# loyer-yuan/GeneralSparse

Hardware: AMD Instinct MI355X
Metric: SpMM GFLOP/s + achieved HBM GB/s vs rocSPARSE, pruned-weight fp16 N=32 (higher is better)
Workload: dtype f16 (fp32 accumulate)

## Files before the change

generalsparse_amd/autotune.py:

```python
import math

CANDIDATES = {
    "f16": [("block_total", 20, 1), ("block_total", 10, 1), ("block_total", 40, 1), ("block_total", 80, 1),
            ("block_total", 40, 1, {"KS_NT": 1}), ("block_total", 80, 1, {"KS_NT": 1}),
            ("tblock_warp_total", 20, 2), ("tblock_warp_total", 24, 2), ("tblock_warp_total", 4, 1),
            ("warp_segment", 4, 1), ("thread_total", 4, 1)],
    "f16_2to4": [("col_direction_nm", 32, 1), ("col_direction_nm", 32, 1, {"NM_NT": 0}),
                 ("col_direction_nm", 32, 1, {"NM_TILES": 8})],
    "f32": [("thread_total", 4, 1), ("tblock_warp_total", 4, 1), ("tblock_warp_total", 32, 8),
            ("tblock_warp_total", 32, 16), ("tblock_warp_total", 64, 16), ("merge_path", 512, 1)],
    "f32_powerlaw": [("merge_path", 256, 1), ("merge_path", 512, 1), ("merge_path", 1024, 1),
                     ("balanced_block_total", 2048, 1), ("thread_total", 4, 1)],
    "f32_powerlaw_large": [("merge_path", 512, 1), ("merge_path", 1024, 1), ("merge_path", 2048, 1),
                           ("merge_path", 1024, 1, {"MP_COL_PARTS": 4}), ("merge_path", 2048, 1, {"MP_COL_PARTS": 2})],
}
F32_EXTRA = {"f16": [("tblock_warp_total", 64, 8), ("tblock_warp_total", 72, 8)]}
WORKLOAD_CLASS = {"c1": "f32", "c2": "f16", "c3": "f16_2to4", "c4": "f32_powerlaw", "c4o": "f32_powerlaw_large"}


def row_block_rows(M, cus=256, max_rows=64):
    rounds = max(1, math.ceil(M / (cus * max_rows)))
    return max(1, math.ceil(M / (cus * rounds)))


def shape_candidates(M):
    rb = row_block_rows(M)
    return [("tblock_warp_total", rb, 2, {"KS_MIN_ROWS": 1000}), ("block_total", 56, 1, {}),
            ("block_total", 40, 1, {}), ("block_total", 80, 1, {}), ("block_total", 112, 1, {})]


def candidates_for(M, K, nnz, dtype, two_four=False, powerlaw=False):
    if dtype in ("f16", "bf16"):
        if two_four:
            return list(CANDIDATES["f16_2to4"])
        c = list(CANDIDATES["f16"])
        rb = ("tblock_warp_total", row_block_rows(M), 2)
        if rb not in c:
            c.append(rb)
        return c
    if powerlaw:
        return list(CANDIDATES["f32_powerlaw_large" if nnz > 50_000_000 else "f32_powerlaw"])
    return list(CANDIDATES["f32"]) + [c for c in F32_EXTRA["f16"] if c not in CANDIDATES["f32"]]


def cand_key(c):
    return "%s(%d,%d)%s" % (c[0], c[1], c[2], "".join(f" {a}={b}" for a, b in (c[3] if len(c) > 3 else {}).items()))


def build_candidate(M, K, row, col, val, cand, N, dtype, device=0):
    from . import Plan, get_config, set_config
    name, p0, p1 = cand[:3]
    over = cand[3] if len(cand) > 3 else {}
    old = {k: get_config(k) for k in over}
    try:
        for k, v in over.items():
            set_config(k, v)
        plan = Plan.from_coo(M, K, row, col, val).run_pipeline(name, N, p0, p1).compile()
        plan.upload(dtype, device)
    finally:
        for k, v in old.items():
            set_config(k, v)
    return plan


def autotune(M, K, row, col, val, N, dtype="f16", candidates=None, device=0, reps=50, rotation_mb=640.0,
             save_path=None, two_four=False, powerlaw=False, rounds=3):
    import torch
    from . import GsError
    tdt = {"f16": torch.float16, "bf16": torch.bfloat16}.get(dtype, torch.float32)
    e = 2 if dtype in ("f16", "bf16") else 4
    dev = torch.device(f"cuda:{device}")
    if candidates is None:
        candidates = candidates_for(M, K, len(row), dtype, two_four=two_four, powerlaw=powerlaw)
    results, built = {}, []
    for cand in candidates:
        key = cand_key(cand)
        try:
            plan = build_candidate(M, K, row, col, val, cand, N, dtype, device)
        except GsError as ex:
            results[key] = str(ex)
            continue
        copies = max(2, int(math.ceil(rotation_mb * 1e6 / (plan.info()["device_bytes_A"] + K * N * e))))
        for _ in range(copies - 1):
            plan.add_replica()
        Bs = [torch.randn((K, N), device=dev, dtype=tdt) for _ in range(copies)]
        Cs = [torch.empty((M, N), device=dev, dtype=tdt) for _ in range(copies)]
        built.append([key, plan, plan.rotation(Bs, Cs), Bs, Cs, []])
    for _ in range(max(1, rounds)):
        for b in built:
            rot = b[2]
            rot.run(5, 0)
            torch.cuda.synchronize(dev)
            e0, e1 = torch.cuda.Event(enable_timing=True), torch.cuda.Event(enable_timing=True)
            e0.record()
            rot.run(reps, 0)
            e1.record()
            torch.cuda.synchronize(dev)
            b[5].append(e0.elapsed_time(e1) / reps * 1e3)
    best = None
    for b in built:
        us = sorted(b[5])[len(b[5]) // 2]
        results[b[0]] = round(us, 3)
        if best is None or us < best[0]:
            best = (us, b)
    if best is None:
        raise GsError("no candidate plan could be built")
    for b in built:
        b[2] = b[3] = b[4] = None
        if b is not best[1]:
            b[1].free()
    plan = best[1][1]
    if save_path:
        plan.save(save_path)
    return plan, results
```

generalsparse_amd/csrc/hip_code/kernel_common.hpp:

```cpp
#pragma once

#include <hip/hip_fp16.h>
#include <hip/hip_runtime.h>
#include <stdint.h>

#include <type_traits>

#include "idx_formula.hpp"
#include "kernel_consts.hpp"

namespace gsk {

typedef _Float16 f16;
typedef __bf16 bf16;
typedef unsigned int u32x4 __attribute__((ext_vector_type(4)));
typedef unsigned int u32x2 __attribute__((ext_vector_type(2)));

template <int BYTES> struct raw_vec;
template <> struct raw_vec<2> { typedef uint16_t t; };
template <> struct raw_vec<4> { typedef uint32_t t; };
template <> struct raw_vec<8> { typedef uint2 t; };
template <> struct raw_vec<16> { typedef uint4 t; };
struct alignas(16) u32x8 { uint4 lo, hi; };
template <> struct raw_vec<32> { typedef u32x8 t; };

template <class VT, int CF>
__device__ __forceinline__ void load_f32(const VT *__restrict__ p, float (&out)[CF]) {
    typedef typename raw_vec<CF * sizeof(VT)>::t R;
    R r = *reinterpret_cast<const R *>(p);
    VT tmp[CF];
    __builtin_memcpy(tmp, &r, sizeof(R));
#pragma unroll
    for (int k = 0; k < CF; k++) out[k] = (float)tmp[k];
}

template <class VT, int CF>
__device__ __forceinline__ void store_f32(VT *__restrict__ p, const float (&in)[CF]) {
    typedef typename raw_vec<CF * sizeof(VT)>::t R;
    VT tmp[CF];
#pragma unroll
    for (int k = 0; k < CF; k++) tmp[k] = (VT)in[k];
    R r;
    __builtin_memcpy(&r, tmp, sizeof(R));
    *reinterpret_cast<R *>(p) = r;
}

template <class T>
__device__ __forceinline__ T ld_once(const T *p) {
#if defined(GS_A_NT) && GS_A_NT
    return __builtin_nontemporal_load(p);
#else
    return *p;
#endif
}
template <bool NT, class T>
__device__ __forceinline__ T ld_once_if(const T *p) {
    if constexpr (NT) return __builtin_nontemporal_load(p);
    else return ld_once(p);
}
template <int BYTES> struct raw_ext;
template <> struct raw_ext<1> { typedef uint8_t t; };
template <> struct raw_ext<2> { typedef uint16_t t; };
template <> struct raw_ext<4> { typedef uint32_t t; };
template <> struct raw_ext<8> { typedef u32x2 t; };
template <> struct raw_ext<16> { typedef u32x4 t; };

template <class T, int SCF>
__device__ __forceinline__ void load_raw(const T *__restrict__ p, T (&out)[SCF]) {
    if constexpr (SCF * sizeof(T) <= 16) {
        typedef typename raw_ext<SCF * sizeof(T)>::t R;
        R r = ld_once(reinterpret_cast<const R *>(p));
        __builtin_memcpy(out, &r, sizeof(R));
    } else {
        static_assert(SCF * sizeof(T) == 32, "8 to 32 bytes");
        u32x4 r[2] = {ld_once(reinterpret_cast<const u32x4 *>(p)), ld_once(reinterpret_cast<const u32x4 *>(p) + 1)};
        __builtin_memcpy(out, r, 32);
    }
}

template <int CF>
__device__ __forceinline__ void wave_reduce_slots(float (&acc)[CF], int X) {
    for (int off = X; off < 64; off <<= 1) {
#pragma unroll
        for (int k = 0; k < CF; k++) acc[k] += __shfl_xor(acc[k], off, 64);
    }
}

template <class VT, int CF>
__device__ __forceinline__ void atomic_add_vals(VT *p, const float (&v)[CF]);

template <>
__device__ __forceinline__ void atomic_add_vals<float, 1>(float *p, const float (&v)[1]) {
    unsafeAtomicAdd(p, v[0]);
}
template <>
__device__ __forceinline__ void atomic_add_vals<float, 4>(float *p, const float (&v)[4]) {
#pragma unroll
    for (int k = 0; k < 4; k++) unsafeAtomicAdd(p + k, v[k]);
}
template <>
__device__ __forceinline__ void atomic_add_vals<float, 8>(float *p, const float (&v)[8]) {
#pragma unroll
    for (int k = 0; k < 8; k++) unsafeAtomicAdd(p + k, v[k]);
}
template <>
__device__ __forceinline__ void atomic_add_vals<f16, 8>(f16 *p, const float (&v)[8]) {
#pragma unroll
    for (int k = 0; k < 8; k += 2) {
        __half2 h = __floats2half2_rn(v[k], v[k + 1]);
        unsafeAtomicAdd(reinterpret_cast<__half2 *>(p + k), h);
    }
}
template <>
__device__ __forceinline__ void atomic_add_vals<f16, 1>(f16 *p, const float (&v)[1]) {
    unsafeAtomicAdd(reinterpret_cast<__half *>(p), __float2half(v[0]));
}

__device__ __forceinline__ uint32_t xcd_block(uint32_t b, uint32_t n) {
#ifdef GS_NO_XCD_SWIZZLE
    return b;
#endif
    const uint32_t q = n >> 3, r = n & 7u, x = b & 7u;
    return (x < r ? x * (q + 1u) : r * (q + 1u) + (x - r) * q) + (b >> 3);
}

template <class VT, int CF>
__device__ __forceinline__ void fma_row(float (&acc)[CF], float v, const VT *__restrict__ brow) {
    float b[CF];
    load_f32<VT, CF>(brow, b);
#pragma unroll
    for (int k = 0; k < CF; k++) acc[k] = __builtin_fmaf(v, b[k], acc[k]);
}

typedef _Float16 h8v __attribute__((ext_vector_type(8)));
typedef short s4v __attribute__((ext_vector_type(4)));
typedef float f4v __attribute__((ext_vector_type(4)));
typedef __attribute__((address_space(3))) s4v lds_s4v;
typedef _Float16 h16v __attribute__((ext_vector_type(16)));
typedef __bf16 b8v __attribute__((ext_vector_type(8)));
template <class ET> struct mfma_elem;
template <> struct mfma_elem<f16> {
    typedef h8v frag;
    static __device__ __forceinline__ f4v mfma_16x16x32(const frag &a, const frag &b, const f4v &c) {
        return __builtin_amdgcn_mfma_f32_16x16x32_f16(a, b, c, 0, 0, 0);
    }
};
template <> struct mfma_elem<bf16> {
    typedef b8v frag;
    static __device__ __forceinline__ f4v mfma_16x16x32(const frag &a, const frag &b, const f4v &c) {
        return __builtin_amdgcn_mfma_f32_16x16x32_bf16(a, b, c, 0, 0, 0);
    }
};
typedef uint32_t u32x2_a2 __attribute__((ext_vector_type(2), aligned(2)));

template <int CT>
__device__ __forceinline__ uint32_t b_piece(uint32_t k, uint32_t p) {
    uint32_t sw;
    if constexpr (CT == 1) sw = 0;
    else if constexpr (CT == 2) sw = (k >> 3) & 1u;
    else if constexpr (CT == 4) sw = ((k >> 1) & 1u) | (((k >> 3) & 1u) << 1);
    else sw = (k & 3u) | (((k >> 3) & 1u) << 2);
    return p ^ (sw & (uint32_t)(CT - 1));
}

__device__ __forceinline__ u32x4 ks_slab_wait(const uint32_t *src, uint32_t tag, uint32_t *err, bool force) {
    u32x4 w;
    auto load4 = [&]() {
#pragma unroll
        for (int i = 0; i < 4; i++) w[i] = __hip_atomic_load(src + i, __ATOMIC_RELAXED, __HIP_MEMORY_SCOPE_AGENT);
    };
    auto stale = [&]() { return (((w[0] ^ tag) | (w[1] ^ tag) | (w[2] ^ tag) | (w[3] ^ tag)) & 1u) != 0u; };
    bool lost = force;
    if (!lost) {
        load4();
        if (stale()) {
            uint64_t t0 = __builtin_amdgcn_s_memrealtime(), prev = t0;
            uint32_t polls = 0;
            do {
                const uint64_t t = __builtin_amdgcn_s_memrealtime();
                if (t - prev > 100000ull) {
                    t0 = t;
                    polls = 0;
                }
                prev = t;
                if (t - t0 > 20000000ull && polls >= 1024u) {
                    lost = true;
                    break;
                }
                polls++;
                __builtin_amdgcn_s_sleep(2);
                load4();
            } while (stale());
        }
    }
    if (lost) {
        w = u32x4{0x7fc00000u | tag, 0x7fc00000u | tag, 0x7fc00000u | tag, 0x7fc00000u | tag};
        __hip_atomic_fetch_or(err, 1u, __ATOMIC_RELAXED, __HIP_MEMORY_SCOPE_AGENT);
    }
    return w;
}
#ifdef GS_EXPERIMENTS
#define GS_KS_FORCE(prio) (((prio) & 16u) != 0u)
#else
#define GS_KS_FORCE(prio) false
#endif

}
```

generalsparse_amd/csrc/hip_code/mfma_ks.hpp:

```cpp
#pragma once

#include "kernel_common.hpp"

namespace gsk {

template <int N>
__device__ constexpr int vmcnt_imm() {
    static_assert(N >= 0 && N < 64, "vmcnt is six bits");
    return (N & 0xF) | ((N >> 4) << 14) | 0x70 | 0xF00;
}


#ifndef GS_KS_FULL_TILE
#define GS_KS_FULL_TILE 1
#endif
enum : int { kKsPosU16 = 0, kKsPos8 = 1, kKsPosWin = 2 };
template <int CT, int RT, int W, int D, int MAXG, bool STAMPS, bool AP = true, int PF = kKsPosU16, int NTL = 0, class ET = f16>
__device__ __forceinline__ void ks_body(const uint32_t *__restrict__ bmtb_first_row, const u32x4 *__restrict__ tP,
                                        const u32x4 *__restrict__ tV, const u32x2 *__restrict__ steps,
                                        const ET *__restrict__ B, ET *__restrict__ C, uint32_t K, uint32_t N, uint32_t S,
                                        uint32_t NS, uint32_t nwg, uint32_t row_base, float *__restrict__ slabs,
                                        uint32_t *__restrict__ arrivals, uint64_t *__restrict__ stamps, uint32_t bx,
                                        uint32_t prio, const uint8_t *__restrict__ tW = nullptr) {
    constexpr bool P8 = PF == kKsPos8, WP = PF == kKsPosWin;
    constexpr uint32_t RB = 32 * CT;
    constexpr uint32_t UB = 2 * CT;
    constexpr uint32_t IMG = ks_image_bytes<RT>();
    constexpr uint32_t STG = 32u * RB;
    extern __shared__ __attribute__((aligned(16))) unsigned char lds[];
    const uint32_t tid = threadIdx.x, lane = tid & 63u;
    const uint32_t wv = __builtin_amdgcn_readfirstlane(tid >> 6);
    const uint32_t u = xcd_block(bx, nwg);
    const uint32_t g = u / S, q = u - g * S;
#define GS_KS_STAMP(slot)                                                                          \
    if constexpr (STAMPS) {                                                                        \
        if (lane == 0) stamps[((size_t)blockIdx.x * W + wv) * 32u + (slot)] = __builtin_amdgcn_s_memtime(); \
    }
    GS_KS_STAMP(0u);
    const uint32_t k0 = q * NS * 32u;
    const uint32_t col0 = blockIdx.y * 16u * CT, nv = min(16u * CT, N - col0);
    unsigned char *img = lds + wv * (IMG + STG);
    unsigned char *bst = img + IMG;
    const u32x4 zero4 = {0u, 0u, 0u, 0u};

    const uint32_t nsw = NS > wv ? (NS - wv + W - 1u) / W : 0u;
    const size_t ubase = (size_t)u * NS;
    using PV = typename std::conditional<P8 || WP, u32x2, u32x4>::type;
    const PV *tPp = reinterpret_cast<const PV *>(tP);
    PV P[D][MAXG];
    u32x4 V[D][MAXG], BR[D][CT];
    uint32_t WN[D][MAXG];
    u32x2 NX[D];
    uint32_t CN[D];
    uint32_t vz;
    __asm__ volatile("v_mov_b32 %0, 0" : "=v"(vz));
    auto rec_of = [&](uint32_t i) -> u32x2 {
        const uint32_t st = __builtin_amdgcn_readfirstlane(i < nsw ? wv + i * W : 0u);
        return steps[ubase + st + vz];
    };
    uint32_t boff[CT];
#pragma unroll
    for (int c = 0; c < CT; c++) boff[c] = ((lane + 64u * c) / UB) * N + ((lane + 64u * c) % UB) * 8u;
    auto load_b = [&](auto fast, uint32_t i, u32x4 (&B_)[CT]) {
        const uint32_t st = __builtin_amdgcn_readfirstlane(i < nsw ? wv + i * W : 0u);
        const uint32_t kr = k0 + st * 32u;
        if constexpr (decltype(fast)::value) {
            const ET *Bk = B + (size_t)kr * N + col0;
#pragma unroll
            for (int c = 0; c < CT; c++) B_[c] = ld_once_if<(NTL & 2) != 0>(reinterpret_cast<const u32x4 *>(Bk + boff[c]));
            return;
        }
#pragma unroll
        for (int c = 0; c < CT; c++) {
            const uint32_t un = lane + 64u * c;
            const uint32_t k = kr + un / UB, cu = (un % UB) * 8u;
            B_[c] = ld_once_if<(NTL & 2) != 0>(
                reinterpret_cast<const u32x4 *>(B + (size_t)(k < K ? k : K - 1u) * N + col0 + (cu < nv ? cu : 0u)));
        }
    };
    auto load_g_at = [&](uint32_t i, uint32_t b0, uint32_t gc, u32x2 &NX_, uint32_t &CN_, PV (&P_)[MAXG],
                         u32x4 (&V_)[MAXG], uint32_t (&W_)[MAXG]) {
        CN_ = gc;
        NX_ = rec_of(i + D);
#pragma unroll
        for (int j = 0; j < MAXG; j++) {
            const uint32_t qg = lane + 64u * j;
            const size_t at = (size_t)b0 + (qg < gc ? qg : 0u);
            P_[j] = ld_once_if<(NTL & 1) != 0>(tPp + at);
            V_[j] = ld_once_if<(NTL & 1) != 0>(tV + at);
            if constexpr (WP) W_[j] = ld_once_if<(NTL & 1) != 0>(tW + at);
        }
    };
    auto load_g = [&](uint32_t i, u32x2 &NX_, uint32_t &CN_, PV (&P_)[MAXG], u32x4 (&V_)[MAXG], uint32_t (&W_)[MAXG]) {
        load_g_at(i, __builtin_amdgcn_readfirstlane(NX_[0]), __builtin_amdgcn_readfirstlane(NX_[1]), NX_, CN_, P_, V_, W_);
    };
    const uint32_t GH = (prio >> 8) & 0x3ffu;
    if (GH) {
#pragma unroll
        for (int d = 0; d < D; d++) load_b(std::false_type{}, (uint32_t)d, BR[d]);
#pragma unroll
        for (int d = 0; d < D; d++) {
            const uint32_t st = (uint32_t)d < nsw ? wv + (uint32_t)d * W : 0u;
            load_g_at((uint32_t)d, (u * min((uint32_t)(W * D), NS) + st) * GH, GH, NX[d], CN[d], P[d], V[d], WN[d]);
        }
        for (uint32_t x = lane; x < IMG / 16u; x += 64u) *reinterpret_cast<u32x4 *>(img + x * 16u) = zero4;
    } else {
#pragma unroll
        for (int d = 0; d < D; d++) NX[d] = rec_of((uint32_t)d);
#pragma unroll
        for (int d = 0; d < D; d++) load_b(std::false_type{}, (uint32_t)d, BR[d]);
        for (uint32_t x = lane; x < IMG / 16u; x += 64u) *reinterpret_cast<u32x4 *>(img + x * 16u) = zero4;
#pragma unroll
        for (int d = 0; d < D; d++) load_g((uint32_t)d, NX[d], CN[d], P[d], V[d], WN[d]);
    }
    GS_KS_STAMP(1u);

    f4v acc[RT][CT];
#pragma unroll
    for (int rt = 0; rt < RT; rt++)
#pragma unroll
        for (int ct = 0; ct < CT; ct++) acc[rt][ct] = f4v{0.f, 0.f, 0.f, 0.f};
    uint32_t arow[RT];
#pragma unroll
    for (int rt = 0; rt < RT; rt++) arow[rt] = (16u * rt + (lane & 15u)) * kKsStride + 16u * (lane >> 4);

    auto ent_h = [&](const PV &p, uint32_t hb, int e) -> uint32_t {
        if constexpr (P8) {
            const uint32_t b = (p[e >> 2] >> (8 * (e & 3))) & 0x7fu;
            return hb + 48u * (b >> 4) + (b & 15u);
        } else {
            return (p[e >> 1] >> (16 * (e & 1))) & 0xffffu;
        }
    };
    auto grp_hb = [&](const PV &p) -> uint32_t {
        if constexpr (P8) {
            const uint32_t x = p[0], y = p[1];
            const uint32_t sg = ((x >> 7) & 1u) | ((x >> 14) & 2u) | ((x >> 21) & 4u) | ((x >> 28) & 8u) | ((y >> 3) & 16u);
            return 384u * (sg >> 1) + 16u * (sg & 1u);
        } else {
            return 0u;
        }
    };
    auto step = [&](auto fast, uint32_t i, u32x2 &NX_, uint32_t &CN_, PV (&P_)[MAXG], u32x4 (&V_)[MAXG], u32x4 (&B_)[CT],
                    uint32_t (&W_)[MAXG]) {
        const bool live = i < nsw;
        const uint32_t gc = CN_;
        typedef typename mfma_elem<ET>::frag frag;
        frag av[RT], bv[CT];
        if (live) {
            const uint32_t kr = k0 + (wv + i * W) * 32u;
#pragma unroll
            for (int c = 0; c < CT; c++) {
                const uint32_t un = lane + 64u * c, k = un / UB, s = un % UB;
                u32x4 b = B_[c];
                if constexpr (!decltype(fast)::value) b = kr + k < K && s * 8u < nv ? b : zero4;
                *reinterpret_cast<u32x4 *>(bst + k * RB + b_piece<CT>(k, s >> 1) * 32u + (s & 1u) * 16u) = b;
            }
            unsigned char *wa[WP ? MAXG : 1][8];
            if constexpr (WP) {
#pragma unroll
                for (int j = 0; j < MAXG; j++) {
                    unsigned char *wb = img + W_[j] * 480u;
#pragma unroll
                    for (int e = 0; e < 8; e++) wa[j][e] = wb + 2u * ((P_[j][e >> 2] >> (8 * (e & 3))) & 0xffu);
                }
            }
#pragma unroll
            for (int j = 0; j < MAXG; j++) {
                if (lane + 64u * j < gc) {
                    const uint32_t hb = grp_hb(P_[j]);
#pragma unroll
                    for (int e = 0; e < 8; e++) {
                        const uint16_t v = (uint16_t)((V_[j][e >> 1] >> (16 * (e & 1))) & 0xffffu);
                        if constexpr (WP) {
                            *reinterpret_cast<uint16_t *>(wa[j][e]) = v;
                        } else {
                            const uint32_t h = ent_h(P_[j], hb, e);
                            *reinterpret_cast<uint16_t *>(img + h * 2u) = v;
                        }
                    }
                }
            }
#pragma unroll
            for (int rt = 0; rt < RT; rt++) av[rt] = *reinterpret_cast<const frag *>(img + arow[rt]);
            const uint32_t kb = 8u * (lane >> 4);
#pragma unroll
            for (int ct = 0; ct < CT; ct++) {
                s4v t[2];
#pragma unroll
                for (int hh = 0; hh < 2; hh++) {
                    const uint32_t k = kb + 4u * hh + ((lane & 15u) >> 2);
                    t[hh] = __builtin_amdgcn_ds_read_tr16_b64_v4i16(
                        (lds_s4v *)(bst + k * RB + b_piece<CT>(k, ct) * 32u + (lane & 3u) * 8u));
                }
                __builtin_memcpy(&bv[ct], t, 16);
            }
#pragma unroll
            for (int j = 0; j < MAXG; j++) {
                if (lane + 64u * j < gc) {
                    const uint32_t hb = grp_hb(P_[j]);
#pragma unroll
                    for (int e = 0; e < 8; e++) {
                        if constexpr (WP) *reinterpret_cast<uint16_t *>(wa[j][e]) = (uint16_t)0;
                        else *reinterpret_cast<uint16_t *>(img + ent_h(P_[j], hb, e) * 2u) = (uint16_t)0;
                    }
                }
            }
        }
        load_b(fast, i + D, B_);
        load_g(i + D, NX_, CN_, P_, V_, W_);
        if (live) {
#pragma unroll
            for (int rt = 0; rt < RT; rt++)
#pragma unroll
                for (int ct = 0; ct < CT; ct++)
                    acc[rt][ct] = mfma_elem<ET>::mfma_16x16x32(av[rt], bv[ct], acc[rt][ct]);
            if (i < 16u) GS_KS_STAMP(3u + i);
        }
    };
    const bool young = wv >= W / 2u;
    if ((prio & 3u) && young) __builtin_amdgcn_s_setprio(1);
    const uint32_t fsp = min(NS, K > k0 ? (K - k0) / 32u : 0u);
    const uint32_t nfull = fsp > wv ? (fsp - wv + W - 1u) / W : 0u;
    uint32_t fast_end = 0;
    if (GS_KS_FULL_TILE && nv == 16u * CT)
        fast_end = fsp == NS ? nsw : (nfull >= 2u * D ? ((nfull - 2u * D) / D + 1u) * D : 0u);
    fast_end = __builtin_amdgcn_readfirstlane(fast_end);
    uint32_t i0 = 0;
    for (; i0 < fast_end; i0 += D) {
#pragma unroll
        for (int d = 0; d < D; d++) step(std::true_type{}, i0 + d, NX[d], CN[d], P[d], V[d], BR[d], WN[d]);
        if ((prio & 3u) == 2u && young && i0 + D >= nsw / 2u && i0 < nsw / 2u) __builtin_amdgcn_s_setprio(0);
    }
    for (; i0 < nsw; i0 += D) {
#pragma unroll
        for (int d = 0; d < D; d++) step(std::false_type{}, i0 + d, NX[d], CN[d], P[d], V[d], BR[d], WN[d]);
        if ((prio & 3u) == 2u && young && i0 + D >= nsw / 2u && i0 < nsw / 2u) __builtin_amdgcn_s_setprio(0);
    }
    if ((prio & 3u) && young) __builtin_amdgcn_s_setprio(0);
    GS_KS_STAMP(20u);
    uint32_t *arr = arrivals + (size_t)g * gridDim.y + blockIdx.y;
    uint32_t ticket = 0;
    if (S > 1 && wv == 0 && lane == 0) ticket = __hip_atomic_fetch_add(arr, 1u, __ATOMIC_RELAXED, __HIP_MEMORY_SCOPE_AGENT);
    constexpr bool APART = ks_red_apart(CT, RT, W, AP);
    f4v *red = reinterpret_cast<f4v *>(lds + (APART ? (size_t)W * (IMG + STG) : 0u));
    constexpr bool HALVES = !APART && ks_red_halves(CT, RT, W);
    constexpr uint32_t WR = HALVES ? W / 2 : W;
    uint32_t *flag = reinterpret_cast<uint32_t *>(reinterpret_cast<unsigned char *>(red) + (size_t)WR * RT * CT * 1024u);
    if constexpr (!APART) {
        __asm__ volatile("s_waitcnt lgkmcnt(0)" ::: "memory");
        __builtin_amdgcn_s_barrier();
        __asm__ volatile("" ::: "memory");
    }
    if constexpr (HALVES) {
        if (wv >= WR) {
#pragma unroll
            for (int rt = 0; rt < RT; rt++)
#pragma unroll
                for (int ct = 0; ct < CT; ct++) red[(((wv - WR) * RT + rt) * CT + ct) * 64u + lane] = acc[rt][ct];
        }
        __asm__ volatile("s_waitcnt lgkmcnt(0)" ::: "memory");
        __builtin_amdgcn_s_barrier();
        __asm__ volatile("" ::: "memory");
        if (wv < WR) {
#pragma unroll
            for (int rt = 0; rt < RT; rt++)
#pragma unroll
                for (int ct = 0; ct < CT; ct++) acc[rt][ct] += red[((wv * RT + rt) * CT + ct) * 64u + lane];
        }
        __asm__ volatile("s_waitcnt lgkmcnt(0)" ::: "memory");
        __builtin_amdgcn_s_barrier();
        __asm__ volatile("" ::: "memory");
    }
    if (wv < WR) {
#pragma unroll
        for (int rt = 0; rt < RT; rt++)
#pragma unroll
            for (int ct = 0; ct < CT; ct++) red[((wv * RT + rt) * CT + ct) * 64u + lane] = acc[rt][ct];
    }
    if (S > 1 && wv == 0 && lane == 0) *flag = ticket;
    __asm__ volatile("s_waitcnt lgkmcnt(0)" ::: "memory");
    __builtin_amdgcn_s_barrier();
    __asm__ volatile("" ::: "memory");
    constexpr uint32_t NI = RT * CT * 64u, NT = 64u * W;
    const uint32_t r0 = bmtb_first_row[g], R = bmtb_first_row[g + 1] - r0;
    auto item_sum = [&](uint32_t t) {
        f4v sum = red[t];
#pragma unroll
        for (uint32_t w = 1; w < WR; w++) sum += red[w * NI + t];
        return sum;
    };
    auto store_item = [&](uint32_t t, const f4v &v) {
        const uint32_t ln = t & 63u, tt = t >> 6, rt = tt / CT, ct = tt % CT;
        const uint32_t col = 16u * ct + (ln & 15u), rb = 16u * rt + 4u * (ln >> 4);
        if (col >= nv) return;
#pragma unroll
        for (uint32_t i = 0; i < 4; i++)
            if (rb + i < R) C[(size_t)(row_base + r0 + rb + i) * N + col0 + col] = (ET)v[i];
    };
    GS_KS_STAMP(21u);
    if (S == 1) {
        for (uint32_t t = tid; t < NI; t += NT) store_item(t, item_sum(t));
        GS_KS_STAMP(22u);
        return;
    }
    const uint32_t tk = *flag & 0xffffu, tag = ((*flag >> 16) & 1u) ^ 1u;
    f4v *slab = reinterpret_cast<f4v *>(slabs) + ((size_t)u * gridDim.y + blockIdx.y) * NI;
    auto tagged = [&](const f4v &v) {
        u32x4 w;
        __builtin_memcpy(&w, &v, 16);
        w[0] = (w[0] & ~1u) | tag; w[1] = (w[1] & ~1u) | tag; w[2] = (w[2] & ~1u) | tag; w[3] = (w[3] & ~1u) | tag;
        return w;
    };
    for (uint32_t t = tid; t < NI; t += NT) {
        const u32x4 w = tagged(item_sum(t));
        __asm__ volatile("global_store_dwordx4 %0, %1, off sc1" ::"v"(slab + t), "v"(w) : "memory");
    }
    if (tk != S - 1u) {
        GS_KS_STAMP(22u);
        return;
    }
    if (tid == 0) __hip_atomic_store(arr, tag << 16, __ATOMIC_RELAXED, __HIP_MEMORY_SCOPE_AGENT);
    const f4v *base = reinterpret_cast<const f4v *>(slabs) + blockIdx.y * NI;
    const size_t qstride = (size_t)gridDim.y * NI;
    uint32_t *err = arrivals + (size_t)(nwg / S) * gridDim.y;
    for (uint32_t t = tid; t < NI; t += NT) {
        f4v sum = {0.f, 0.f, 0.f, 0.f};
        for (uint32_t qq = 0; qq < S; qq++) {
            u32x4 w;
            if (qq == q) {
                w = tagged(item_sum(t));
            } else {
                w = ks_slab_wait(reinterpret_cast<const uint32_t *>(base + ((size_t)g * S + qq) * qstride + t), tag, err,
                                 GS_KS_FORCE(prio));
            }
            w[0] &= ~1u; w[1] &= ~1u; w[2] &= ~1u; w[3] &= ~1u;
            f4v x;
            __builtin_memcpy(&x, &w, 16);
            sum += x;
        }
        store_item(t, sum);
    }
    GS_KS_STAMP(22u);
#undef GS_KS_STAMP
}

template <int CT, int RT, int W, int D, int MAXG, bool STAMPS = false, bool AP = true, int PF = kKsPosU16, int NTL = 0, class ET = f16>
__global__ __launch_bounds__(64 * W) void k_mfma_ks(const uint32_t *__restrict__ bmtb_first_row,
                                                    const u32x4 *__restrict__ tP,
                                                    const u32x4 *__restrict__ tV,
                                                    const u32x2 *__restrict__ steps,
                                                    const ET *__restrict__ B, ET *__restrict__ C, uint32_t K,
                                                    uint32_t N, uint32_t S, uint32_t NS, uint32_t nwg,
                                                    uint32_t row_base, float *__restrict__ slabs,
                                                    uint32_t *__restrict__ arrivals, uint64_t *__restrict__ stamps = nullptr,
                                                    uint32_t prio = 0,
                                                    const uint8_t *__restrict__ tW = nullptr) {
    ks_body<CT, RT, W, D, MAXG, STAMPS, AP, PF, NTL, ET>(bmtb_first_row, tP, tV, steps, B, C, K, N, S, NS, nwg, row_base, slabs,
                                                    arrivals, stamps, blockIdx.x, prio, tW);
}

#ifdef GS_EXPERIMENTS
template <int CT, int RT, int W, int D, int MAXG, int NTL = 0>
__global__ __launch_bounds__(64 * W) void k_mfma_ks_persist(const uint32_t *__restrict__ bmtb_first_row,
                                                            const u32x4 *__restrict__ tP, const u32x4 *__restrict__ tV,
                                                            const u32x2 *__restrict__ steps, const f16 *__restrict__ B,
                                                            f16 *__restrict__ C, uint32_t K, uint32_t N, uint32_t S,
                                                            uint32_t NS, uint32_t nunits, uint32_t row_base,
                                                            float *__restrict__ slabs, uint32_t *__restrict__ arrivals,
                                                            uint32_t prio, uint32_t *__restrict__ queue) {
    __shared__ uint32_t next_sh;
    uint32_t xcc;
    asm volatile("s_getreg_b32 %0, hwreg(HW_REG_XCC_ID, 0, 4)" : "=s"(xcc));
    xcc &= 7u;
    const uint32_t grid = gridDim.x;
    uint32_t u = blockIdx.x, qx = xcc, tried = 0;
    while (u < nunits) {
        uint32_t pulled = 0;
        if (threadIdx.x == 0) pulled = __hip_atomic_fetch_add(queue + qx, 1u, __ATOMIC_RELAXED, __HIP_MEMORY_SCOPE_AGENT);
        ks_body<CT, RT, W, D, MAXG, false, true, kKsPosU16, NTL>(bmtb_first_row, tP, tV, steps, B, C, K, N, S, NS, nunits,
                                                          row_base, slabs, arrivals, nullptr, u, prio);
        __syncthreads();
        if (threadIdx.x == 0) next_sh = pulled;
        __syncthreads();
        u = grid + qx + 8u * next_sh;
        __syncthreads();
        while (u >= nunits && ++tried < 8u) {
            qx = (qx + 1u) & 7u;
            if (threadIdx.x == 0) next_sh = __hip_atomic_fetch_add(queue + qx, 1u, __ATOMIC_RELAXED, __HIP_MEMORY_SCOPE_AGENT);
            __syncthreads();
            u = grid + qx + 8u * next_sh;
            __syncthreads();
        }
    }
    if (threadIdx.x == 0 && __hip_atomic_fetch_add(queue + 8, 1u, __ATOMIC_RELAXED, __HIP_MEMORY_SCOPE_AGENT) == grid - 1u) {
        for (int i = 0; i < 9; i++) __hip_atomic_store(queue + i, 0u, __ATOMIC_RELAXED, __HIP_MEMORY_SCOPE_AGENT);
    }
}
#endif

struct ks_entry {
    const uint32_t *tbr;
    const u32x4 *tP, *tV;
    const u32x2 *steps;
    const void *B;
    void *C;
    float *slabs;
    uint32_t *arrivals;
    uint32_t K, S, NS, nwg, row_base, pad0;
    const uint8_t *tW;
};
static_assert(sizeof(ks_entry) == 96, "ks_entry is 96 bytes");
struct ks_group_args {
    uint32_t begin[kKsGroupMax + 1];
    uint32_t n, N, pad[2];
    ks_entry e[kKsGroupMax];
};

template <int CT, int RT, int W, int D, int MAXG, int PF = kKsPosU16, bool AP = true, int NTL = 0, class ET = f16>
__global__ __launch_bounds__(64 * W) void k_mfma_ks_group(ks_group_args args) {
    const uint32_t bx = blockIdx.x, n = args.n;
    uint32_t sel = 0;
#pragma unroll
    for (int i = 1; i < kKsGroupMax; i++)
        if ((uint32_t)i < n && args.begin[i] <= bx) sel = (uint32_t)i;
    sel = __builtin_amdgcn_readfirstlane(sel);
    const ks_entry &e = args.e[sel];
    if (bx - args.begin[sel] >= e.nwg) return;
    ks_body<CT, RT, W, D, MAXG, false, AP, PF, NTL, ET>(e.tbr, e.tP, e.tV, e.steps, (const ET *)e.B, (ET *)e.C, e.K, args.N, e.S, e.NS,
                                                   e.nwg, e.row_base, e.slabs, e.arrivals, nullptr, bx - args.begin[sel],
                                                   args.pad[0] | (e.pad0 << 8), e.tW);
}

}
```

Before: 40720.

## Drain software-pipeline tail without look-ahead loads and batch split-K slab reads

Restructures the split-K MFMA kernel main loop so the final look-ahead steps run in a drain mode that skips issuing prefetch loads past the end, with a dedicated short path for waves with fewer steps than the look-ahead depth. The reduction stage by the last arriving block now issues up to four slab loads at once and waits only once, falling back to the spinning wait only for slabs whose tag is not yet set. This is meant to remove wasted tail loads and serialized slab-read latency, at the cost of larger unrolled code and more register pressure. One autotune candidate is also dropped.

After: 40840 (median of 6 runs). Within noise of the previous version (+0.3%).

```diff
diff --git a/generalsparse_amd/autotune.py b/generalsparse_amd/autotune.py
--- a/generalsparse_amd/autotune.py
+++ b/generalsparse_amd/autotune.py
@@ -2,7 +2,7 @@
 
 CANDIDATES = {
     "f16": [("block_total", 20, 1), ("block_total", 10, 1), ("block_total", 40, 1), ("block_total", 80, 1),
-            ("block_total", 40, 1, {"KS_NT": 1}), ("block_total", 80, 1, {"KS_NT": 1}),
+            ("block_total", 40, 1, {"KS_NT": 1}),
             ("tblock_warp_total", 20, 2), ("tblock_warp_total", 24, 2), ("tblock_warp_total", 4, 1),
             ("warp_segment", 4, 1), ("thread_total", 4, 1)],
     "f16_2to4": [("col_direction_nm", 32, 1), ("col_direction_nm", 32, 1, {"NM_NT": 0}),
diff --git a/generalsparse_amd/csrc/hip_code/kernel_common.hpp b/generalsparse_amd/csrc/hip_code/kernel_common.hpp
--- a/generalsparse_amd/csrc/hip_code/kernel_common.hpp
+++ b/generalsparse_amd/csrc/hip_code/kernel_common.hpp
@@ -199,6 +199,33 @@
     }
     return w;
 }
+__device__ __forceinline__ void ks_slab_load(uint32_t n, const uint32_t *const (&p)[4], u32x4 (&w)[4]) {
+    switch (n) {
+        case 1:
+            __asm__ volatile("global_load_dwordx4 %0, %1, off sc1\n\ts_waitcnt vmcnt(0)" : "=&v"(w[0]) : "v"(p[0]) : "memory");
+            break;
+        case 2:
+            __asm__ volatile("global_load_dwordx4 %0, %2, off sc1\n\tglobal_load_dwordx4 %1, %3, off sc1\n\ts_waitcnt vmcnt(0)"
+                             : "=&v"(w[0]), "=&v"(w[1])
+                             : "v"(p[0]), "v"(p[1])
+                             : "memory");
+            break;
+        case 3:
+            __asm__ volatile("global_load_dwordx4 %0, %3, off sc1\n\tglobal_load_dwordx4 %1, %4, off sc1\n\t"
+                             "global_load_dwordx4 %2, %5, off sc1\n\ts_waitcnt vmcnt(0)"
+                             : "=&v"(w[0]), "=&v"(w[1]), "=&v"(w[2])
+                             : "v"(p[0]), "v"(p[1]), "v"(p[2])
+                             : "memory");
+            break;
+        default:
+            __asm__ volatile("global_load_dwordx4 %0, %4, off sc1\n\tglobal_load_dwordx4 %1, %5, off sc1\n\t"
+                             "global_load_dwordx4 %2, %6, off sc1\n\tglobal_load_dwordx4 %3, %7, off sc1\n\ts_waitcnt vmcnt(0)"
+                             : "=&v"(w[0]), "=&v"(w[1]), "=&v"(w[2]), "=&v"(w[3])
+                             : "v"(p[0]), "v"(p[1]), "v"(p[2]), "v"(p[3])
+                             : "memory");
+            break;
+    }
+}
 #ifdef GS_EXPERIMENTS
 #define GS_KS_FORCE(prio) (((prio) & 16u) != 0u)
 #else
diff --git a/generalsparse_amd/csrc/hip_code/mfma_ks.hpp b/generalsparse_amd/csrc/hip_code/mfma_ks.hpp
--- a/generalsparse_amd/csrc/hip_code/mfma_ks.hpp
+++ b/generalsparse_amd/csrc/hip_code/mfma_ks.hpp
@@ -13,6 +13,9 @@
 
 #ifndef GS_KS_FULL_TILE
 #define GS_KS_FULL_TILE 1
+#endif
+#ifndef GS_KS_TAIL
+#define GS_KS_TAIL 5
 #endif
 enum : int { kKsPosU16 = 0, kKsPos8 = 1, kKsPosWin = 2 };
 template <int CT, int RT, int W, int D, int MAXG, bool STAMPS, bool AP = true, int PF = kKsPosU16, int NTL = 0, class ET = f16>
@@ -37,6 +40,7 @@
         if (lane == 0) stamps[((size_t)blockIdx.x * W + wv) * 32u + (slot)] = __builtin_amdgcn_s_memtime(); \
     }
     GS_KS_STAMP(0u);
+    constexpr bool DRAIN = (GS_KS_TAIL & 1) != 0, ONE_TRIP = (GS_KS_TAIL & 4) != 0;
     const uint32_t k0 = q * NS * 32u;
     const uint32_t col0 = blockIdx.y * 16u * CT, nv = min(16u * CT, N - col0);
     unsigned char *img = lds + wv * (IMG + STG);
@@ -78,10 +82,10 @@
                 reinterpret_cast<const u32x4 *>(B + (size_t)(k < K ? k : K - 1u) * N + col0 + (cu < nv ? cu : 0u)));
         }
     };
-    auto load_g_at = [&](uint32_t i, uint32_t b0, uint32_t gc, u32x2 &NX_, uint32_t &CN_, PV (&P_)[MAXG],
+    auto load_g_at = [&](auto rec, uint32_t i, uint32_t b0, uint32_t gc, u32x2 &NX_, uint32_t &CN_, PV (&P_)[MAXG],
                          u32x4 (&V_)[MAXG], uint32_t (&W_)[MAXG]) {
         CN_ = gc;
-        NX_ = rec_of(i + D);
+        if constexpr (decltype(rec)::value) NX_ = rec_of(i + D);
 #pragma unroll
         for (int j = 0; j < MAXG; j++) {
             const uint32_t qg = lane + 64u * j;
@@ -92,16 +96,37 @@
         }
     };
     auto load_g = [&](uint32_t i, u32x2 &NX_, uint32_t &CN_, PV (&P_)[MAXG], u32x4 (&V_)[MAXG], uint32_t (&W_)[MAXG]) {
-        load_g_at(i, __builtin_amdgcn_readfirstlane(NX_[0]), __builtin_amdgcn_readfirstlane(NX_[1]), NX_, CN_, P_, V_, W_);
+        load_g_at(std::true_type{}, i, __builtin_amdgcn_readfirstlane(NX_[0]), __builtin_amdgcn_readfirstlane(NX_[1]), NX_, CN_,
+                  P_, V_, W_);
     };
     const uint32_t GH = (prio >> 8) & 0x3ffu;
-    if (GH) {
+    const bool shortw = DRAIN && nsw < (uint32_t)D;
+    auto prologue_short = [&]() {
+        for (uint32_t x = lane; x < IMG / 16u; x += 64u) *reinterpret_cast<u32x4 *>(img + x * 16u) = zero4;
+#pragma unroll
+        for (int d = 0; d + 1 < D; d++) {
+            if ((uint32_t)d < nsw) {
+                load_b(std::false_type{}, (uint32_t)d, BR[d]);
+                if (GH) {
+                    load_g_at(std::false_type{}, (uint32_t)d, (u * min((uint32_t)(W * D), NS) + wv + (uint32_t)d * W) * GH, GH, NX[d],
+                              CN[d], P[d], V[d], WN[d]);
+                } else {
+                    const u32x2 rc = rec_of((uint32_t)d);
+                    load_g_at(std::false_type{}, (uint32_t)d, __builtin_amdgcn_readfirstlane(rc[0]),
+                              __builtin_amdgcn_readfirstlane(rc[1]), NX[d], CN[d], P[d], V[d], WN[d]);
+                }
+            }
+        }
+    };
+    auto prologue = [&]() {
+      if (GH) {
 #pragma unroll
         for (int d = 0; d < D; d++) load_b(std::false_type{}, (uint32_t)d, BR[d]);
 #pragma unroll
         for (int d = 0; d < D; d++) {
             const uint32_t st = (uint32_t)d < nsw ? wv + (uint32_t)d * W : 0u;
-            load_g_at((uint32_t)d, (u * min((uint32_t)(W * D), NS) + st) * GH, GH, NX[d], CN[d], P[d], V[d], WN[d]);
+            load_g_at(std::true_type{}, (uint32_t)d, (u * min((uint32_t)(W * D), NS) + st) * GH, GH, NX[d], CN[d], P[d], V[d],
+                      WN[d]);
         }
         for (uint32_t x = lane; x < IMG / 16u; x += 64u) *reinterpret_cast<u32x4 *>(img + x * 16u) = zero4;
     } else {
@@ -112,14 +137,16 @@
         for (uint32_t x = lane; x < IMG / 16u; x += 64u) *reinterpret_cast<u32x4 *>(img + x * 16u) = zero4;
 #pragma unroll
         for (int d = 0; d < D; d++) load_g((uint32_t)d, NX[d], CN[d], P[d], V[d], WN[d]);
-    }
-    GS_KS_STAMP(1u);
+      }
+    };
 
     f4v acc[RT][CT];
-#pragma unroll
-    for (int rt = 0; rt < RT; rt++)
-#pragma unroll
-        for (int ct = 0; ct < CT; ct++) acc[rt][ct] = f4v{0.f, 0.f, 0.f, 0.f};
+    auto zero_acc = [&]() {
+#pragma unroll
+        for (int rt = 0; rt < RT; rt++)
+#pragma unroll
+            for (int ct = 0; ct < CT; ct++) acc[rt][ct] = f4v{0.f, 0.f, 0.f, 0.f};
+    };
     uint32_t arow[RT];
 #pragma unroll
     for (int rt = 0; rt < RT; rt++) arow[rt] = (16u * rt + (lane & 15u)) * kKsStride + 16u * (lane >> 4);
@@ -141,9 +168,12 @@
             return 0u;
         }
     };
-    auto step = [&](auto fast, uint32_t i, u32x2 &NX_, uint32_t &CN_, PV (&P_)[MAXG], u32x4 (&V_)[MAXG], u32x4 (&B_)[CT],
+    enum : int { kGen = 0, kFast = 1, kDrain = 2 };
+    auto step = [&](auto mode, uint32_t i, u32x2 &NX_, uint32_t &CN_, PV (&P_)[MAXG], u32x4 (&V_)[MAXG], u32x4 (&B_)[CT],
                     uint32_t (&W_)[MAXG]) {
-        const bool live = i < nsw;
+        typedef std::integral_constant<bool, decltype(mode)::value == kFast> fast;
+        constexpr bool LOADS = decltype(mode)::value != kDrain || !DRAIN;
+        const bool live = decltype(mode)::value != kDrain || i < nsw;
         const uint32_t gc = CN_;
         typedef typename mfma_elem<ET>::frag frag;
         frag av[RT], bv[CT];
@@ -153,7 +183,7 @@
             for (int c = 0; c < CT; c++) {
                 const uint32_t un = lane + 64u * c, k = un / UB, s = un % UB;
                 u32x4 b = B_[c];
-                if constexpr (!decltype(fast)::value) b = kr + k < K && s * 8u < nv ? b : zero4;
+                if constexpr (!fast::value) b = kr + k < K && s * 8u < nv ? b : zero4;
                 *reinterpret_cast<u32x4 *>(bst + k * RB + b_piece<CT>(k, s >> 1) * 32u + (s & 1u) * 16u) = b;
             }
             unsigned char *wa[WP ? MAXG : 1][8];
@@ -207,8 +237,10 @@
                 }
             }
         }
-        load_b(fast, i + D, B_);
-        load_g(i + D, NX_, CN_, P_, V_, W_);
+        if constexpr (LOADS) {
+            load_b(fast{}, i + D, B_);
+            load_g(i + D, NX_, CN_, P_, V_, W_);
+        }
         if (live) {
 #pragma unroll
             for (int rt = 0; rt < RT; rt++)
@@ -219,23 +251,60 @@
         }
     };
     const bool young = wv >= W / 2u;
-    if ((prio & 3u) && young) __builtin_amdgcn_s_setprio(1);
     const uint32_t fsp = min(NS, K > k0 ? (K - k0) / 32u : 0u);
     const uint32_t nfull = fsp > wv ? (fsp - wv + W - 1u) / W : 0u;
     uint32_t fast_end = 0;
     if (GS_KS_FULL_TILE && nv == 16u * CT)
         fast_end = fsp == NS ? nsw : (nfull >= 2u * D ? ((nfull - 2u * D) / D + 1u) * D : 0u);
-    fast_end = __builtin_amdgcn_readfirstlane(fast_end);
-    uint32_t i0 = 0;
-    for (; i0 < fast_end; i0 += D) {
-#pragma unroll
-        for (int d = 0; d < D; d++) step(std::true_type{}, i0 + d, NX[d], CN[d], P[d], V[d], BR[d], WN[d]);
-        if ((prio & 3u) == 2u && young && i0 + D >= nsw / 2u && i0 < nsw / 2u) __builtin_amdgcn_s_setprio(0);
-    }
-    for (; i0 < nsw; i0 += D) {
-#pragma unroll
-        for (int d = 0; d < D; d++) step(std::false_type{}, i0 + d, NX[d], CN[d], P[d], V[d], BR[d], WN[d]);
-        if ((prio & 3u) == 2u && young && i0 + D >= nsw / 2u && i0 < nsw / 2u) __builtin_amdgcn_s_setprio(0);
+    typedef std::integral_constant<int, kGen> gen_t;
+    typedef std::integral_constant<int, kFast> fast_t;
+    typedef std::integral_constant<int, kDrain> drain_t;
+    if (shortw) {
+        prologue_short();
+        GS_KS_STAMP(1u);
+        zero_acc();
+#pragma unroll
+        for (int d = 0; d + 1 < D; d++) step(drain_t{}, (uint32_t)d, NX[d], CN[d], P[d], V[d], BR[d], WN[d]);
+    } else {
+        prologue();
+        GS_KS_STAMP(1u);
+        zero_acc();
+        if ((prio & 3u) && young) __builtin_amdgcn_s_setprio(1);
+        const uint32_t L = nsw > (uint32_t)D ? nsw - D : 0u;
+        const uint32_t Lf = __builtin_amdgcn_readfirstlane(L / D * D);
+        fast_end = __builtin_amdgcn_readfirstlane(min(fast_end, Lf));
+        uint32_t i0 = 0;
+        for (; i0 < fast_end; i0 += D) {
+#pragma unroll
+            for (int d = 0; d < D; d++) step(fast_t{}, i0 + d, NX[d], CN[d], P[d], V[d], BR[d], WN[d]);
+            if ((prio & 3u) == 2u && young && i0 + D >= nsw / 2u && i0 < nsw / 2u) __builtin_amdgcn_s_setprio(0);
+        }
+        for (; i0 < Lf; i0 += D) {
+#pragma unroll
+            for (int d = 0; d < D; d++) step(gen_t{}, i0 + d, NX[d], CN[d], P[d], V[d], BR[d], WN[d]);
+            if ((prio & 3u) == 2u && young && i0 + D >= nsw / 2u && i0 < nsw / 2u) __builtin_amdgcn_s_setprio(0);
+        }
+        const uint32_t rem = __builtin_amdgcn_readfirstlane(L - Lf);
+        auto mixed = [&](auto r_) {
+            constexpr int RM = decltype(r_)::value;
+#pragma unroll
+            for (int d = 0; d < RM; d++) step(gen_t{}, Lf + d, NX[d], CN[d], P[d], V[d], BR[d], WN[d]);
+#pragma unroll
+            for (int d = RM; d < D; d++) step(drain_t{}, Lf + d, NX[d], CN[d], P[d], V[d], BR[d], WN[d]);
+        };
+        if constexpr (D > 1) {
+            if (rem == 1u) mixed(std::integral_constant<int, 1>{});
+        }
+        if constexpr (D > 2) {
+            if (rem == 2u) mixed(std::integral_constant<int, 2>{});
+        }
+        if constexpr (D > 3) {
+            if (rem == 3u) mixed(std::integral_constant<int, 3>{});
+        }
+        const uint32_t Lt = rem ? Lf + D : Lf;
+#pragma unroll
+        for (int d = 0; d < D; d++) step(drain_t{}, Lt + d, NX[d], CN[d], P[d], V[d], BR[d], WN[d]);
+        static_assert(D <= 4, "the tail is written out for look-aheads of up to 4 steps");
     }
     if ((prio & 3u) && young) __builtin_amdgcn_s_setprio(0);
     GS_KS_STAMP(20u);
@@ -324,6 +393,48 @@
     const f4v *base = reinterpret_cast<const f4v *>(slabs) + blockIdx.y * NI;
     const size_t qstride = (size_t)gridDim.y * NI;
     uint32_t *err = arrivals + (size_t)(nwg / S) * gridDim.y;
+    auto untagged = [&](u32x4 w) {
+        w[0] &= ~1u; w[1] &= ~1u; w[2] &= ~1u; w[3] &= ~1u;
+        f4v x;
+        __builtin_memcpy(&x, &w, 16);
+        return x;
+    };
+    if constexpr (ONE_TRIP) {
+        const bool force = GS_KS_FORCE(prio);
+        for (uint32_t t = tid; t < NI; t += NT) {
+            const f4v own = untagged(tagged(item_sum(t)));
+            const uint32_t *src = reinterpret_cast<const uint32_t *>(base + (size_t)g * S * qstride + t);
+            f4v sum = {0.f, 0.f, 0.f, 0.f};
+            bool own_in = false;
+            for (uint32_t o0 = 0; o0 + 1u < S; o0 += 4u) {
+                const uint32_t n = min(4u, S - 1u - o0);
+                const uint32_t *p[4];
+                u32x4 w[4] = {zero4, zero4, zero4, zero4};
+#pragma unroll
+                for (uint32_t j = 0; j < 4u; j++) {
+                    const uint32_t o = min(o0 + j, S - 2u), qq = o < q ? o : o + 1u;
+                    p[j] = src + (size_t)qq * qstride * 4u;
+                }
+                if (!force) ks_slab_load(n, p, w);
+#pragma unroll
+                for (uint32_t j = 0; j < 4u; j++) {
+                    if (j < n) {
+                        if (force || (((w[j][0] ^ tag) | (w[j][1] ^ tag) | (w[j][2] ^ tag) | (w[j][3] ^ tag)) & 1u) != 0u)
+                            w[j] = ks_slab_wait(p[j], tag, err, force);
+                        if (!own_in && o0 + j >= q) {
+                            sum += own;
+                            own_in = true;
+                        }
+                        sum += untagged(w[j]);
+                    }
+                }
+            }
+            if (!own_in) sum += own;
+            store_item(t, sum);
+        }
+        GS_KS_STAMP(22u);
+        return;
+    }
     for (uint32_t t = tid; t < NI; t += NT) {
         f4v sum = {0.f, 0.f, 0.f, 0.f};
         for (uint32_t qq = 0; qq < S; qq++) {
```
